# genjax-dev/genjax

Measured on AMD Instinct MI355X. Metric: particles/sec (particle-steps/s), bootstrap SMC sweep, linear-Gaussian SSM T=100, higher is better.
Workload: dtype f32; 1 GPU; BASELINE config 2: linear-Gaussian state-space (T=100), bootstrap SMC, systematic resampling every step; particles_per_gpu=1000000, particles_total=1000000, T=100, resampler=systematic, graph=True, key=314159

## Files before the change

### genjax_amd/csrc/gmx_jit.h

```cpp
#pragma once
#include "gmx_block.h"
#include "gmx_vm.h"
#include "gmx_peer.h"
#if defined(GMX_JIT_RS)
#include "gmx_offspring.h"
#endif
#if defined(GMX_JIT_SH)
#include "gmx_shard_fill.h"
#endif

#if defined(GMX_JIT_BACKGROUND)
#define GMX_JIT_PRIO
#define GMX_JIT_NAME gmx_jit_background_kernel
#else
#define GMX_JIT_PRIO GMX_SETPRIO
#define GMX_JIT_NAME gmx_jit_kernel
#endif

#if defined(GMX_JIT_RS_LOOP)
#define GMX_JIT_BLK gmx_blk
#define GMX_RS_LOOP_MAX 16
#else
#define GMX_JIT_BLK blockIdx.x
#endif

template <int NDYN, int PPV>
struct gmx_jit_ctx {
  const uint32_t* consts;
  const gmx_run_args* A;
  float* lds4;
  uint64_t* lds8;
  float red_x[PPV];
  int cur;
  uint32_t blk;
  uint32_t part;
  uint32_t rows;
  int64_t n_rows;
  float acc_max;
  uint64_t* peer_land;
  uint32_t peer_tag;
  bool first, last;
  __device__ __forceinline__ uint32_t pool(uint32_t i) const {
    return i < (uint32_t)NDYN ? A->uni[i] : consts[i - (uint32_t)NDYN];
  }
  __device__ __forceinline__ const void* in_ptr(uint32_t s) const { return A->in_d[s]; }
  __device__ __forceinline__ void* out_ptr(uint32_t s) const { return A->out_d[s]; }
  __device__ __forceinline__ const void* tab_ptr(uint32_t s) const { return A->tab_d[s]; }
  __device__ __forceinline__ void red_max(float x, bool active) {
    const float m = active ? x : -gmx_inf();
    red_x[cur] = m;
    acc_max = first ? m : gmx_rmax(acc_max, m);
    if (last) {
      const float bm = block_max(acc_max, lds4);
      if (threadIdx.x == 0 && A->red_out_d) A->red_out_d[blk] = bm;
      if (PPV == 4 && A->tile_agg_d) {
        const float ref = gmx_tile_ref(gmx_tile_exp(bm));
        uint64_t s = 0;
#pragma unroll
        for (int p = 0; p < PPV; ++p) s += gmx_exp_fixed(red_x[p] - ref, A->tile_shift);
        s = wave_sum_u64(s);
        if ((threadIdx.x & 63) == 0) lds8[threadIdx.x >> 6] = s;
        __syncthreads();
        const uint64_t a_b = (lds8[0] + lds8[1]) + (lds8[2] + lds8[3]);
        if (threadIdx.x == 0) A->tile_agg_d[blk] = a_b;
        if (peer_land) gmx_peer_put_tile(peer_land, peer_tag, A->peer.world, A->peer.tiles, A->peer.rank, (int)blk, a_b, bm);
      }
    }
  }
  __device__ __forceinline__ void red_lse(float x, bool active) {
    gmx_red_lse(A->red_out_d, lds4, part, rows, x, active);
  }
};

#if defined(GMX_JIT_SH)
#define GMX_JIT_OCC __attribute__((amdgpu_waves_per_eu(1, 4)))
#else
#define GMX_JIT_OCC
#endif
#if defined(GMX_JIT_RS_LOOP)
#define GMX_JIT_LOOP_OPEN                                                                        \
    const int gmx_tiles = (int)((n + (int64_t)(PP * GMX_BLOCK) - 1) / (int64_t)(PP * GMX_BLOCK)); \
    const int gmx_G = (int)gridDim.x;                                                            \
    const int gmx_C = (gmx_tiles + gmx_G - 1) / gmx_G;                                           \
    if (PP == 4 && A.rs.lw_d) {                                                                  \
      __shared__ uint64_t gmx_pf[GMX_RS_LOOP_MAX];                                               \
      uint64_t gmx_tot, gmx_mk;                                                                  \
      gmx_tile_table_pass(A.rs.tile_max_d, A.rs.tile_agg_d, gmx_tiles, (int)blockIdx.x, gmx_G, gmx_C, gmx_pf, gmx_tot, gmx_mk); \
      GMX_JIT_NOUNROLL for (int gmx_c = 0; gmx_c < gmx_C; ++gmx_c) {                             \
        const int gmx_tile = (int)blockIdx.x + gmx_c * gmx_G;                                    \
        if (gmx_tile < gmx_tiles)                                                                \
          gmx_offspring_tile_body<GMX_RESAMPLE_SYSTEMATIC, 0, true>(A.rs.key0, A.rs.key1, A.rs.u0, A.rs.lw_d, A.rs.tile_max_d, \
              (const uint64_t*)nullptr, n, gmx_tiles, gmx_pow2i(A.rs.shift), A.rs.max_out_d, A.rs.total_out_d, \
              const_cast<int32_t*>(A.ancestors_d), nullptr, A.rs.tag, gmx_tile, gmx_pf[gmx_c], gmx_tot, gmx_mk); \
        __syncthreads();                                                                         \
      }                                                                                          \
    }                                                                                            \
    GMX_JIT_NOUNROLL for (int gmx_lc = 0; gmx_lc < gmx_C; ++gmx_lc) {                            \
      const uint32_t gmx_blk = blockIdx.x + (uint32_t)gmx_lc * (uint32_t)gmx_G;                  \
      if ((int)gmx_blk >= gmx_tiles) break;                                   \
      if (gmx_lc) __syncthreads();
#define GMX_JIT_LOOP_CLOSE }
#else
#define GMX_JIT_LOOP_OPEN
#define GMX_JIT_LOOP_CLOSE
#endif
#define GMX_JIT_BEGIN(NREGS, FULLV, NDYN, PPV, NPRE)                                             \
  extern "C" __global__ void __launch_bounds__(GMX_BLOCK) GMX_JIT_OCC GMX_JIT_NAME(int64_t n, const gmx_run_args A) { \
 GMX_JIT_PRIO                                                                                 \
    __shared__ float lds4[4];                                                                    \
    __shared__ uint64_t lds8[4];                                                                 \
    constexpr int PP = PPV;                                                                      \
    typedef gmx_regs_vgpr<NREGS> regs_t;                                                         \
    typedef gmx_jit_ctx<NDYN, PPV> ctx_t;                                                        \
    constexpr bool full_v = FULLV;                                                               \
    ctx_t ctx;                                                                                   \
    ctx.consts = GMX_JIT_CONST; ctx.A = &A; ctx.lds4 = lds4; ctx.lds8 = lds8; ctx.part = 0; ctx.cur = 0; \
    ctx.rows = (uint32_t)((n + GMX_BLOCK - 1) / GMX_BLOCK); ctx.n_rows = n;      \
    ctx.peer_land = nullptr; ctx.peer_tag = 0u;                                                  \
    if (PPV == 4 && A.peer.land_d) {                                         \
      ctx.peer_tag = *A.peer.tag_base_d + (uint32_t)A.peer.step;                                 \
      if (threadIdx.x < (uint32_t)A.peer.world && (int)threadIdx.x != A.peer.rank)               \
        ctx.peer_land = (uint64_t*)A.peer.land_d[threadIdx.x];                                   \
    }                                                                                            \
    GMX_JIT_LOOP_OPEN                                                                            \
    ctx.blk = GMX_JIT_BLK;                                                                       \
    regs_t R[PP];                                                                                \
      \
    const uint32_t n32 = (uint32_t)n;                                                            \
    int64_t idx[PP];                                                                             \
    uint32_t cidx[PP];          \
    uint32_t arow[PP];                                                      \
    uint32_t pre[(NPRE) > 0 ? (NPRE) : 1][PP];                                                   \
    bool act[PP];                                                                                \
    uint32_t gmx_t = 0u;        \
    uint32_t gmx_t0 = 0u, gmx_tf = 0u;    \
               \
    const uint32_t row0 = blockIdx.y * n32;                                                      \
    _Pragma("unroll") for (int p = 0; p < PP; ++p) {                                             \
      R[p].init();                                                                               \
      const uint32_t i32 = (GMX_JIT_BLK * (uint32_t)PP + (uint32_t)p) * (uint32_t)GMX_BLOCK + threadIdx.x; \
      idx[p] = (int64_t)(row0 + i32);                                                            \
      act[p] = i32 < n32;                                                                        \
      cidx[p] = row0 + (act[p] ? i32 : n32 - 1u);                                                \
      arow[p] = 0u;                                                                              \
    }                                                                                            \
    (void)cidx; (void)arow; (void)pre; (void)gmx_t; (void)gmx_t0; (void)gmx_tf;

#define GMX_JIT_POLL_ANC(TAG, STATUS, LIMIT)                                                     \
      const uint32_t* gmx_aw = reinterpret_cast<const uint32_t*>(A.ancestors_d);                 \
      uint32_t gmx_av[PP];                                                                       \
      bool gmx_ok = true;                                                                        \
      _Pragma("unroll") for (int p = 0; p < PP; ++p) {                                           \
        gmx_av[p] = __hip_atomic_load(gmx_aw + cidx[p], __ATOMIC_RELAXED, __HIP_MEMORY_SCOPE_AGENT); \
        gmx_ok &= (gmx_av[p] >> GMX_ANC_TAG_SHIFT) == (TAG);                                     \
      }                                                                                          \
      if (!gmx_ok) {                                                                             \
        const uint64_t gmx_t0 = wall_clock64();                                                  \
        do {                                                                                     \
          __builtin_amdgcn_s_sleep(1);                                                           \
          gmx_ok = true;                                                                         \
          _Pragma("unroll") for (int p = 0; p < PP; ++p) {                                       \
            gmx_av[p] = __hip_atomic_load(gmx_aw + cidx[p], __ATOMIC_RELAXED, __HIP_MEMORY_SCOPE_AGENT); \
            gmx_ok &= (gmx_av[p] >> GMX_ANC_TAG_SHIFT) == (TAG);                                 \
          }                                                                                      \
        } while (!gmx_ok && wall_clock64() - gmx_t0 < 200000000ull);                             \
        if (!gmx_ok) __hip_atomic_store((STATUS), 1ull, __ATOMIC_RELAXED, __HIP_MEMORY_SCOPE_AGENT); \
      }                                                                                          \
      _Pragma("unroll") for (int p = 0; p < PP; ++p) {                                           \
        const uint32_t gmx_i = gmx_av[p] & GMX_ANC_INDEX_MASK;                                   \
        arow[p] = gmx_i < (LIMIT) ? gmx_i : (LIMIT) - 1u;                                        \
      }

#if defined(GMX_JIT_SH)
#define GMX_JIT_PRE_ANC                                                                          \
    if (PP == 4 && A.sh.lw_d) {                                                                  \
      shard_peer gmx_sp;                                                                         \
      gmx_sp.land = (uint64_t* const*)A.sh.peer.land_d; gmx_sp.tag_base = A.sh.peer.tag_base_d;  \
      gmx_sp.status = A.sh.peer.status_d; gmx_sp.step = A.sh.peer.step; gmx_sp.leaves = A.sh.peer.leaves; \
      gmx_sp.state = (const uint32_t* const*)A.sh.state_d; gmx_sp.tail = (uint32_t* const*)A.sh.tail_d;   \
      gmx_shard_fill_body<GMX_RESAMPLE_SYSTEMATIC, true, true, true>(                            \
          A.sh.key0, A.sh.key1, A.sh.u0, A.sh.lw_d, (const uint8_t*)A.sh.stats_own_d, (size_t)0, A.sh.peer.tiles, \
          gmx_pow2i(A.sh.shift), A.sh.peer.rank, A.sh.peer.world, (int32_t)n, (int32_t)A.sh.peer.capacity, A.sh.plan_d, \
          A.sh.total_out_d, A.sh.max_out_d, (const uint32_t*)nullptr, (uint32_t*)nullptr,         \
          const_cast<int32_t*>(A.ancestors_d), gmx_sp, A.sh.tag);                                 \
      const uint32_t gmx_lim = n32 + (uint32_t)A.sh.peer.world * (uint32_t)A.sh.peer.capacity;   \
      GMX_JIT_POLL_ANC(A.sh.tag, A.sh.status_d, gmx_lim)                                         \
       \
    } else {                                                                                     \
      _Pragma("unroll") for (int p = 0; p < PP; ++p) arow[p] = (uint32_t)A.ancestors_d[cidx[p]]; \
    }
#elif defined(GMX_JIT_RS_LOOP)
#define GMX_JIT_PRE_ANC                                                                          \
    if (PP == 4 && A.rs.lw_d) {                                                                  \
      GMX_JIT_POLL_ANC(A.rs.tag, A.rs.status_d, n32)                                             \
    } else {                                                                                     \
      _Pragma("unroll") for (int p = 0; p < PP; ++p) arow[p] = (uint32_t)A.ancestors_d[cidx[p]]; \
    }
#elif defined(GMX_JIT_RS)
#define GMX_JIT_PRE_ANC                                                                          \
    if (PP == 4 && A.rs.lw_d) {                                                                  \
      gmx_offspring_tile_body<GMX_RESAMPLE_SYSTEMATIC, 4, true>(A.rs.key0, A.rs.key1, A.rs.u0, A.rs.lw_d, A.rs.tile_max_d, \
          A.rs.tile_agg_d, n, (int)gridDim.x, gmx_pow2i(A.rs.shift), A.rs.max_out_d, A.rs.total_out_d,          \
          const_cast<int32_t*>(A.ancestors_d), nullptr, A.rs.tag);                                \
      GMX_JIT_POLL_ANC(A.rs.tag, A.rs.status_d, n32)                                             \
    } else {                                                                                     \
      _Pragma("unroll") for (int p = 0; p < PP; ++p) arow[p] = (uint32_t)A.ancestors_d[cidx[p]]; \
    }
#else
#define GMX_JIT_PRE_ANC                                                                          \
    _Pragma("unroll") for (int p = 0; p < PP; ++p) arow[p] = (uint32_t)A.ancestors_d[cidx[p]];
#endif

#define GMX_JIT_PRE_LOAD(K, SLOT, U8, ROW)                                                       \
    _Pragma("unroll") for (int p = 0; p < PP; ++p)                                               \
      pre[K][p] = (U8) ? (uint32_t)((const uint8_t*)A.in_d[SLOT])[ROW[p]] : ((const uint32_t*)A.in_d[SLOT])[ROW[p]];
#define GMX_JIT_PRE(K, SLOT, U8) GMX_JIT_PRE_LOAD(K, SLOT, U8, cidx)
#define GMX_JIT_PRE_G(K, SLOT, U8) GMX_JIT_PRE_LOAD(K, SLOT, U8, arow)
#define GMX_JIT_FENCE __builtin_amdgcn_sched_barrier(0);

#define GMX_JIT_LDPRE(DST, K)                                                                    \
    _Pragma("unroll") for (int p = 0; p < PP; ++p) R[p].set(DST, pre[K][p]);

#define GMX_JIT_OP(W0, W1)                                                                       \
    _Pragma("unroll") for (int p = 0; p < PP; ++p) {                                             \
      ctx.part = GMX_JIT_BLK * PP + p; ctx.first = (p == 0); ctx.last = (p == PP - 1); ctx.cur = p; \
      gmx_vm_step<regs_t, full_v, gmx_cword<W0, W1>, ctx_t>(R[p], gmx_cword<W0, W1>(), idx[p], act[p], A, ctx, gmx_t, gmx_tf); \
    }

#define GMX_JIT_NOUNROLL _Pragma("clang loop unroll(disable)")
#define GMX_JIT_LOOP(COUNT) GMX_JIT_NOUNROLL for (gmx_t0 = 0u; gmx_t0 < (COUNT); ++gmx_t0) { gmx_t = gmx_t0; gmx_tf = gmx_t0;
#define GMX_JIT_ENDLOOP } gmx_t = 0u; gmx_t0 = 0u; gmx_tf = 0u;
#define GMX_JIT_LOOP2(COUNT) GMX_JIT_NOUNROLL for (uint32_t gmx_t1 = 0u; gmx_t1 < (COUNT); ++gmx_t1) { gmx_t = gmx_t1; gmx_tf = gmx_t0 * (COUNT) + gmx_t1;
#define GMX_JIT_ENDLOOP2 } gmx_t = gmx_t0; gmx_tf = gmx_t0;
#define GMX_JIT_LOOP3(COUNT) { const uint32_t gmx_tp = gmx_t, gmx_tfp = gmx_tf;                  \
    GMX_JIT_NOUNROLL for (uint32_t gmx_t2 = 0u; gmx_t2 < (COUNT); ++gmx_t2) { gmx_t = gmx_t2; gmx_tf = gmx_tfp * (COUNT) + gmx_t2;
#define GMX_JIT_ENDLOOP3 } gmx_t = gmx_tp; gmx_tf = gmx_tfp; }

#define GMX_JIT_END GMX_JIT_LOOP_CLOSE }
```

### genjax_amd/csrc/gmx_kernels.hip

```cpp
#include <hip/hip_runtime.h>
#include <hip/hiprtc.h>
#include <stdio.h>
#include <stdlib.h>
#include <string.h>
#include <sys/stat.h>
#include <unistd.h>

#include <new>
#include <atomic>
#include <string>
#include <vector>

#include "gmx_block.h"
#include "gmx_vm.h"
#include "gmx_resample.h"
#include "gmx_peer.h"
#include "gmx_sorted.h"
#include "gmx_offspring.h"
#include "gmx_shard_fill.h"

static thread_local char g_err[512] = "";

static int gmx_fail(const char* fmt, const char* a = "", long long b = 0) {
  snprintf(g_err, sizeof(g_err), fmt, a, b);
// ... 144 lines not shown
      case OP_LOOP: ok = loop_depth < 3 && w1 >= 1u; ++loop_depth; in_loop = true; P.uses_loop = true; break;
      case OP_ENDLOOP: ok = loop_depth > 0; --loop_depth; in_loop = loop_depth > 0; break;
      case OP_UNI: ok = D(dst) && w1 < P.n_uni; break;
      case OP_LDIN:
        ok = D(dst) && a < P.n_in && (!(b & GMX_F_IDX) || (R(c) && !(b & (GMX_F_STEP | GMX_F_FLAT | GMX_F_BCAST))));
        if (b & GMX_F_GATHER) P.uses_gather = true;
        break;
      case OP_LDTAB: ok = D(dst) && R(b) && a < P.n_tab; break;
      case OP_STOUT: ok = R(b) && a < P.n_out; break;
      case OP_LDKEY: ok = R2(dst); P.uses_key = true; break;
      case OP_KDERIVE: ok = R2(dst) && R2(a); break;
      case OP_KDERIVER: ok = R2(dst) && R2(a) && R(b); break;
      case OP_KSPLITU: ok = R2(dst) && R(a) && R(b); break;
      case OP_MOV: case OP_NEG: case OP_ABS: case OP_EXP: case OP_LOG: case OP_LOG1P:
      case OP_SQRT: case OP_SIN: case OP_COS: case OP_TANH: case OP_SIGMOID:
      case OP_SOFTPLUS: case OP_FLOOR: case OP_CEIL: case OP_ROUND: case OP_LGAMMA:
      case OP_SQUARE: case OP_RECIP: case OP_NOT: case OP_I2F: case OP_F2I: case OP_INEG:
        ok = D(dst) && R(a); break;
      case OP_ADD: case OP_SUB: case OP_MUL: case OP_DIV: case OP_MIN: case OP_MAX: case OP_POW:
      case OP_FLT: case OP_FLE: case OP_FGT: case OP_FGE: case OP_FEQ: case OP_FNE:
      case OP_IEQ: case OP_INE: case OP_ILT: case OP_ILE: case OP_IGT: case OP_IGE:
      case OP_AND: case OP_OR: case OP_XOR: case OP_IADD: case OP_ISUB: case OP_IMUL:
        ok = D(dst) && R(a) && R(b); break;
      case OP_SEL: ok = D(dst) && R(a) && R(b) && R(c); break;
      case OP_S_NORMAL: case OP_S_UNIFORM: case OP_S_BETA:
        ok = D(dst) && R(a) && R(b) && R2(c); break;
      case OP_S_FLIP: case OP_S_BERNL: case OP_S_LOGGAMMA: ok = D(dst) && R(a) && R2(c); break;
      case OP_S_CATSTEP: ok = R2(dst) && R(a) && R(b) && R2(c); break;
      case OP_L_NORMAL: case OP_L_UNIFORM: case OP_L_BETA:
        ok = D(dst) && R(a) && R(b) && R(c); break;
      case OP_L_FLIP: case OP_L_BERNL: ok = D(dst) && R(a) && R(c); break;
      case OP_REDMAX: case OP_REDLSE:
        ok = R(a); P.uses_red = true;
        if (op == OP_REDLSE) P.uses_lse = true; else ++P.n_redmax;
        break;
      default: ok = false;
    }
    if ((op == OP_LDIN && (b & (GMX_F_STEP | GMX_F_IDX))) || (op == OP_STOUT && (dst & GMX_F_STEP))) {
      P.uses_step = true;
    }
    if (!ok) return gmx_fail("gmx_program_create: invalid instruction%s at pc %lld", "", pc);
  }
  if (in_loop) return gmx_fail("gmx_program_create: OP_LOOP without OP_ENDLOOP%s");
  P.code_h.assign(ins, ins + 2 * (size_t)n_instr);
  P.consts.assign(ins + 2 * (size_t)n_instr, ins + 2 * (size_t)n_instr + n_const);
  return 0;
}

extern "C" int gmx_program_create(const uint32_t* blob, size_t n_words, gmx_program** out) {
  if (!out) return gmx_fail("gmx_program_create: null argument%s");
  gmx_program P;
  if (parse_program(blob, n_words, P)) return 1;
  const uint32_t n_instr = P.n_instr;
  GMX_HIP(hipMalloc((void**)&P.code_d, sizeof(uint32_t) * 2 * (n_instr ? n_instr : 1)));
  if (n_instr)
    GMX_HIP(hipMemcpy(P.code_d, P.code_h.data(), sizeof(uint32_t) * 2 * n_instr, hipMemcpyHostToDevice));
  gmx_program* h = new (std::nothrow) gmx_program(P);
  if (!h) return gmx_fail("gmx_program_create: out of host memory%s");
  *out = h;
  return 0;
}

extern "C" int gmx_program_destroy(gmx_program* p) {
  if (!p) return 0;
  if (p->code_d) (void)hipFree(p->code_d);
  if (p->jit_module) (void)hipModuleUnload(p->jit_module);
  delete p;
  return 0;
}


#include "gmx_embed.inc"

static bool jit_enabled() {
  const char* e = getenv("GENMI_JIT");
  return !(e && e[0] == '0');
}

static int jit_pp_for(const gmx_program* p) {
  return (p->n_regs <= 16 && p->n_instr <= 96 && !p->uses_lse) ? 4 : 1;
}

#define JIT_MAX_PRE 8
static std::string jit_source(const gmx_program* p, bool* gathers_prefetched = nullptr) {
  std::string s = p->background ? "#define GMX_JIT_BACKGROUND 1\n" : "";
  if (const char* f_ = getenv("GENMI_JIT_FAULT")) { if (f_[0] == '1') s += "#define GMX_JIT_FAULT 1\n"; }
  if (p->fuse_rs) s += "#define GMX_JIT_RS 1\n";
  if (p->fuse_rs_loop) s += "#define GMX_JIT_RS_LOOP 1\n";
  if (p->fuse_sh) s += "#define GMX_JIT_SH 1\n";
  s += "#include \"gmx_jit.h\"\n";
  char buf[128];
  s += "__device__ static constexpr uint32_t GMX_JIT_CONST[] = {";
  for (size_t k = 0; k < p->consts.size(); ++k) { snprintf(buf, sizeof(buf), "0x%08xu,", p->consts[k]); s += buf; }
  s += "0u};\n";
  struct pre_t { uint32_t slot, flags; };
  std::vector<pre_t> pres;
  std::vector<int> pre_of(p->n_instr, -1);
  bool any_gather = false;
  uint32_t first_gather_pc = p->n_instr, first_key_pc = p->n_instr;
  bool fits = true, seen_loop = false;
  for (uint32_t pc = 0; pc < p->n_instr && fits; ++pc) {
    const uint32_t w0 = p->code_h[2 * pc], op = w0 & 0xffu, a = (w0 >> 16) & 0xffu, b = w0 >> 24;
    if ((op == OP_LDKEY || op == OP_KDERIVE) && first_key_pc == p->n_instr && !seen_loop) first_key_pc = pc;
    if (op == OP_LOOP) seen_loop = true;
    if (op != OP_LDIN || (b & (GMX_F_BCAST | GMX_F_STEP | GMX_F_IDX))) continue;
    int k = -1;
    for (size_t j = 0; j < pres.size(); ++j)
      if (pres[j].slot == a && pres[j].flags == b) k = (int)j;
    if (k < 0) {
      if (pres.size() == JIT_MAX_PRE) { fits = false; break; }
      k = (int)pres.size();
      pres.push_back({a, b});
    }
    pre_of[pc] = k;
    if (b & GMX_F_GATHER) { any_gather = true; if (pc < first_gather_pc) first_gather_pc = pc; }
  }
  if (const char* e_ = getenv("GENMI_JIT_NOPRE")) { if (e_[0] == '1' && !p->fuse_rs && !p->fuse_sh) fits = false; }
  if (!fits) { pres.clear(); pre_of.assign(p->n_instr, -1); any_gather = false; }
  if (gathers_prefetched) {
    *gathers_prefetched = any_gather;
    for (uint32_t pc = 0; pc < p->n_instr; ++pc) {
      const uint32_t w0 = p->code_h[2 * pc];
      if ((w0 & 0xffu) == OP_LDIN && ((w0 >> 24) & GMX_F_GATHER) && pre_of[pc] < 0) *gathers_prefetched = false;
    }
  }
  const uint32_t gpos = (any_gather && first_key_pc < first_gather_pc) ? first_key_pc + 1 : 0;
  snprintf(buf, sizeof(buf), "GMX_JIT_BEGIN(%u, %s, %u, %d, %d)\n", p->n_regs < 16 ? 16u : (p->n_regs < 32 ? 32u : 64u),
           p->needs_full ? "true" : "false", p->n_dyn, jit_pp_for(p), (int)pres.size());
  s += buf;
  if (any_gather) s += "  GMX_JIT_PRE_ANC\n";
  for (size_t k = 0; k < pres.size(); ++k)
    if (!(pres[k].flags & GMX_F_GATHER)) {
      snprintf(buf, sizeof(buf), "  GMX_JIT_PRE(%d, %u, %d)\n", (int)k, pres[k].slot, (pres[k].flags & GMX_F_U8) ? 1 : 0);
      s += buf;
    }
  auto gathers = [&]() {
    for (size_t k = 0; k < pres.size(); ++k)
      if (pres[k].flags & GMX_F_GATHER) {
        snprintf(buf, sizeof(buf), "  GMX_JIT_PRE_G(%d, %u, %d)\n", (int)k, pres[k].slot, (pres[k].flags & GMX_F_U8) ? 1 : 0);
        s += buf;
      }
    s += "  GMX_JIT_FENCE\n";
  };
  if (!pres.empty()) s += "  GMX_JIT_FENCE\n";
  if (any_gather && gpos == 0) gathers();
  int jit_depth = 0;
  for (uint32_t pc = 0; pc < p->n_instr; ++pc) {
    const uint32_t op_ = p->code_h[2 * pc] & 0xffu;
    if (op_ == OP_LOOP) {
      static const char* const open_[3] = {"  GMX_JIT_LOOP(%uu)\n", "  GMX_JIT_LOOP2(%uu)\n", "  GMX_JIT_LOOP3(%uu)\n"};
      snprintf(buf, sizeof(buf), open_[jit_depth < 2 ? jit_depth : 2], p->code_h[2 * pc + 1]);
      ++jit_depth;
    } else if (op_ == OP_ENDLOOP) {
      static const char* const close_[3] = {"  GMX_JIT_ENDLOOP\n", "  GMX_JIT_ENDLOOP2\n", "  GMX_JIT_ENDLOOP3\n"};
      --jit_depth;
      snprintf(buf, sizeof(buf), "%s", close_[jit_depth < 2 ? (jit_depth < 0 ? 0 : jit_depth) : 2]);
    }
    else if (pre_of[pc] >= 0)
      snprintf(buf, sizeof(buf), "  GMX_JIT_LDPRE(%u, %d)\n", (p->code_h[2 * pc] >> 8) & 0xffu, pre_of[pc]);
    else
      snprintf(buf, sizeof(buf), "  GMX_JIT_OP(0x%08xu, 0x%08xu)\n", p->code_h[2 * pc], p->code_h[2 * pc + 1]);
    s += buf;
    if (any_gather && gpos == pc + 1) gathers();
  }
  s += "GMX_JIT_END\n";
  return s;
}

extern "C" int gmx_program_is_specialized(const gmx_program* p) { return p && p->jit_fn ? 1 : 0; }
static std::atomic<int64_t> g_jit_rejected{0};
extern "C" int64_t gmx_jit_rejected_count(void) { return g_jit_rejected.load(); }
extern "C" int gmx_program_despecialize(gmx_program* p, const char* why) {
  if (!p) return gmx_fail("gmx_program_despecialize: null program%s");
  if (!p->jit_fn) return 0;
  (void)hipDeviceSynchronize();
  (void)hipModuleUnload(p->jit_module);
  p->jit_fn = nullptr; p->jit_module = nullptr; p->jit_code_hash = 0;
  ++g_jit_rejected;
  (void)gmx_fail("specialised kernel rejected, the interpreter takes over: %s", why ? why : "");
  return 0;
}
extern "C" uint64_t gmx_program_code_hash(const gmx_program* p) { return p && p->jit_fn ? p->jit_code_hash : 0ull; }
extern "C" int gmx_program_writes_tile_stats(const gmx_program* p) {
  return p && p->jit_fn && p->jit_pp == 4 && p->n_redmax == 1 && !p->uses_lse ? 1 : 0;
}

extern "C" int gmx_program_set_fuse_resample(gmx_program* p) {
  if (!p) return gmx_fail("gmx_program_set_fuse_resample: null program%s");
  if (p->jit_fn) return gmx_fail("gmx_program_set_fuse_resample: the program is already specialised%s");
  p->fuse_rs = true;
  return 0;
}
extern "C" int gmx_program_set_fuse_resample_loop(gmx_program* p) {
  if (!p) return gmx_fail("gmx_program_set_fuse_resample_loop: null program%s");
  if (p->jit_fn) return gmx_fail("gmx_program_set_fuse_resample_loop: the program is already specialised%s");
  p->fuse_rs = true;
  p->fuse_rs_loop = true;
  return 0;
}
static int64_t rs_loop_grid(const gmx_program* p, int64_t tiles) {
  int64_t g = p->jit_resident_blocks > 0 ? p->jit_resident_blocks : 256;
  if (g > 1024) g = 1024;

  return tiles < g ? tiles : g;
}
extern "C" int gmx_program_fuses_resample(const gmx_program* p) {
  return p && p->jit_fn && p->fuse_rs && p->jit_pp == 4 && p->uses_gather && p->jit_gathers_pre ? 1 : 0;
}
extern "C" int gmx_program_set_fuse_shard_step(gmx_program* p) {
  if (!p) return gmx_fail("gmx_program_set_fuse_shard_step: null program%s");
  if (p->jit_fn) return gmx_fail("gmx_program_set_fuse_shard_step: the program is already specialised%s");
  p->fuse_sh = true;
  return 0;
}
extern "C" int gmx_program_fuses_shard_step(const gmx_program* p) {
  return p && p->jit_fn && p->fuse_sh && p->jit_pp == 4 && p->uses_gather && p->jit_gathers_pre ? 1 : 0;
}
extern "C" int64_t gmx_program_resident_particles(const gmx_program* p) {
// ... 190 lines not shown
  }
  size_t cs = 0;
  if (rc == HIPRTC_SUCCESS) {
    hiprtcGetCodeSize(prog, &cs);
    if (code_out && code_cap >= cs) hiprtcGetCode(prog, code_out);
  }
  hiprtcDestroyProgram(&prog);
  return cs;
}

extern "C" int64_t gmx_program_grid(const gmx_program* p, int64_t n) {
  int64_t per = GMX_BLOCK;
  if (p && p->jit_fn && !p->uses_lse) per = (int64_t)GMX_BLOCK * p->jit_pp;
  return (n + per - 1) / per;
}

static int peer_check(const char* who, const gmx_peer& P, int64_t n_per_rank);
extern "C" int gmx_program_run(const gmx_program* p, int64_t n, const gmx_run_args* args,
                               gmx_stream stream) {
  if (!p || !args) return gmx_fail("gmx_program_run: null argument%s");
  if (n < 0) return gmx_fail("gmx_program_run: negative n%s");
  if (n == 0) return 0;
  if (n > (int64_t)0x7fffffff * GMX_BLOCK) return gmx_fail("gmx_program_run: n too large%s");
  for (uint32_t s = 0; s < p->n_in; ++s)
    if (!args->in_d[s]) return gmx_fail("gmx_program_run: input slot %s%lld is null", "", s);
  for (uint32_t s = 0; s < p->n_out; ++s)
    if (!args->out_d[s]) return gmx_fail("gmx_program_run: output slot %s%lld is null", "", s);
  for (uint32_t s = 0; s < p->n_tab; ++s)
    if (!args->tab_d[s]) return gmx_fail("gmx_program_run: table slot %s%lld is null", "", s);
  if (p->uses_gather && !args->ancestors_d)
    return gmx_fail("gmx_program_run: program gathers but ancestors_d is null%s");
  const bool fused_rs = args->rs.lw_d != nullptr;
  if (fused_rs) {
    const gmx_resample_in& q = args->rs;
    if (!gmx_program_fuses_resample(p))
      return gmx_fail("gmx_program_run: rs is set but this program cannot resample in its own launch "
                      "(gmx_program_set_fuse_resample before specialising; 4 particles per thread; gathering)%s");
    if (!q.tile_max_d || !q.tile_agg_d || !q.max_out_d || !q.total_out_d || !q.status_d)
      return gmx_fail("gmx_program_run: rs has a null pointer%s");
    if ((uintptr_t)q.lw_d & 15) return gmx_fail("gmx_program_run: rs.lw_d must be 16-byte aligned%s");
    if ((!p->fuse_rs_loop && (n + RS_TILE - 1) / RS_TILE > 1024) || n > gmx_program_resident_particles(p) ||
        n > (int64_t)GMX_ANC_INDEX_MASK + 1)
      return gmx_fail("gmx_program_run: rs: every workgroup of the launch must be resident at once (n <= 2^20 and "
                      "n <= gmx_program_resident_particles(); a looped program — gmx_program_set_fuse_resample_loop — "
                      "walks up to 16 tiles per workgroup: n <= 2^24)%s");
    if (q.shift < 1 || q.shift > 62) return gmx_fail("gmx_program_run: rs.shift out of range%s");
    int need = 0;
    while (((int64_t)1 << need) < n) ++need;
    if (q.shift + need > 62) return gmx_fail("gmx_program_run: rs.shift too large for n (overflow)%s");
    if (q.tag < 1u || q.tag > GMX_ANC_TAG_MAX) return gmx_fail("gmx_program_run: rs.tag must be in [1, 255]%s");
    if (args->tile_agg_d == q.tile_agg_d || (const float*)args->red_out_d == q.tile_max_d)
      return gmx_fail("gmx_program_run: rs reads the tile statistics this launch writes (use two sets)%s");
    for (uint32_t s = 0; s < p->n_out; ++s)
      if ((const void*)args->out_d[s] == (const void*)q.lw_d)
        return gmx_fail("gmx_program_run: rs.lw_d is also an output of this launch (use two buffers)%s");
  }
  const bool fused_sh = args->sh.lw_d != nullptr;
  if (fused_sh) {
    const gmx_shard_in& q = args->sh;
    if (fused_rs) return gmx_fail("gmx_program_run: rs and sh are both set%s");
    if (!gmx_program_fuses_shard_step(p))
      return gmx_fail("gmx_program_run: sh is set but this program cannot route a sharded step in its own launch "
                      "(gmx_program_set_fuse_shard_step before specialising; 4 particles per thread; gathering)%s");
    if (!q.stats_own_d || !q.plan_d || !q.total_out_d || !q.max_out_d || !q.status_d)
      return gmx_fail("gmx_program_run: sh has a null pointer%s");
    if (((uintptr_t)q.lw_d & 15) || ((uintptr_t)q.stats_own_d & 7))
      return gmx_fail("gmx_program_run: sh.lw_d must be 16-byte and sh.stats_own_d 8-byte aligned%s");
    if (peer_check("gmx_program_run (sh)", q.peer, n)) return 1;
    if (q.peer.world > 8 || (int64_t)q.peer.world * q.peer.tiles > 4 * GMX_BLOCK)
      return gmx_fail("gmx_program_run: sh: world <= 8 and world * tiles <= 1024%s");
    if (n + (int64_t)q.peer.world * q.peer.capacity > (int64_t)GMX_ANC_INDEX_MASK + 1)
      return gmx_fail("gmx_program_run: sh: n + world * capacity must fit the 21-bit index of an ancestor word%s");
    if (n > gmx_program_resident_particles(p))
      return gmx_fail("gmx_program_run: sh: every workgroup of the launch must be resident at once "
                      "(n <= gmx_program_resident_particles())%s");
    if (q.shift < 1 || q.shift > 62) return gmx_fail("gmx_program_run: sh.shift out of range%s");
    if (q.tag < 1u || q.tag > GMX_ANC_TAG_MAX) return gmx_fail("gmx_program_run: sh.tag must be in [1, 255]%s");
    for (int l = 0; l < q.peer.leaves; ++l)
      if (!q.state_d[l] || !q.tail_d[l]) return gmx_fail("gmx_program_run: sh: a leaf pointer is null%s");
    for (uint32_t s_ = 0; s_ < p->n_out; ++s_)
      if ((const void*)args->out_d[s_] == (const void*)q.lw_d)
        return gmx_fail("gmx_program_run: sh.lw_d is also an output of this launch (use two buffers)%s");
  }
  if (p->uses_red && !args->red_out_d)
    return gmx_fail("gmx_program_run: program reduces but red_out_d is null%s");
  if (args->tile_agg_d) {
    if (!gmx_program_writes_tile_stats(p))
      return gmx_fail("gmx_program_run: tile_agg_d is set but this program cannot write tile statistics "
                      "(gmx_program_writes_tile_stats)%s");
    if (args->tile_shift < 1 || args->tile_shift > 62) return gmx_fail("gmx_program_run: tile_shift out of range%s");
  }
  if (p->uses_step && args->step_stride < n)
    return gmx_fail("gmx_program_run: step_stride must be at least n for a program with step-indexed leaves%s");
  if (p->uses_key) {
    int km = args->key_mode;
    if (km != GMX_KEY_ARRAY && km != GMX_KEY_SPLIT && km != GMX_KEY_ROWSPLIT && km != GMX_KEY_BCAST)
      return gmx_fail("gmx_program_run: program draws but key_mode is unset%s");
    if ((km == GMX_KEY_ARRAY || km == GMX_KEY_ROWSPLIT) && !args->keys_d)
      return gmx_fail("gmx_program_run: keys_d is null%s");
    if (km == GMX_KEY_ROWSPLIT && args->key_inner <= 0)
      return gmx_fail("gmx_program_run: key_inner must be positive%s");
  }
  dim3 grid((unsigned)((n + GMX_BLOCK - 1) / GMX_BLOCK)), block(GMX_BLOCK);
  hipStream_t st = (hipStream_t)stream;
  gmx_run_args patched;
  if (p->n_const || fused_rs || fused_sh) {
    patched = *args;
    for (uint32_t k = 0; k < p->n_const; ++k) patched.uni[p->n_dyn + k] = p->consts[k];
    if (fused_rs) {
      uint32_t b0, b1;
      gmx_threefry2x32(patched.rs.key0, patched.rs.key1, 0u, 0u, &b0, &b1);
      patched.rs.u0 = (b0 ^ b1) >> 9;
    }
    if (fused_sh) {
      uint32_t b0, b1;
      gmx_threefry2x32(patched.sh.key0, patched.sh.key1, 0u, 0u, &b0, &b1);
      patched.sh.u0 = (b0 ^ b1) >> 9;
    }
    args = &patched;
  }
  if (p->jit_fn) {
    if (n >= 0x7fffffffLL - 4 * GMX_BLOCK)
      return gmx_fail("gmx_program_run: a specialised kernel indexes particles with 32 bits (n < 2^31 - 1024)%s");
    struct { int64_t n; gmx_run_args A; } ka;
    ka.n = n; ka.A = *args;
    size_t ka_size = sizeof(ka);
    void* config[] = {HIP_LAUNCH_PARAM_BUFFER_POINTER, &ka, HIP_LAUNCH_PARAM_BUFFER_SIZE, &ka_size,
                      HIP_LAUNCH_PARAM_END};
    int64_t rows = 1, per_row = n;
    if (p->background && args->key_mode == GMX_KEY_ROWSPLIT && args->key_inner > 0 && n % args->key_inner == 0 &&
        n / args->key_inner > 1 && n / args->key_inner <= 65535 && p->n_in == 0 && !p->uses_red && !p->uses_step) {
      rows = n / args->key_inner;
      per_row = args->key_inner;
      ka.n = per_row;
    }
    unsigned jgrid = (unsigned)((per_row + (int64_t)GMX_BLOCK * p->jit_pp - 1) / ((int64_t)GMX_BLOCK * p->jit_pp));
    if (p->fuse_rs_loop && p->jit_pp == 4) jgrid = (unsigned)rs_loop_grid(p, (int64_t)jgrid);
    const unsigned dyn_lds = p->lds_pad;
    GMX_HIP(hipModuleLaunchKernel(p->jit_fn, jgrid, (unsigned)rows, 1, GMX_BLOCK, 1, 1, dyn_lds, st, nullptr, config));
    return 0;
  }
  if (p->n_regs > 31)
    return gmx_fail("gmx_program_run: a program with more than 31 live values runs only as a specialised kernel "
                    "(gmx_program_specialize; hiprtc unavailable or GENMI_JIT=0?)%s");
  if (p->n_regs <= 15) {
    if (p->needs_full)
      hipLaunchKernelGGL((k_vm<gmx_regs_vgpr<16>, true>), grid, block, 0, st, p->code_d, p->n_instr, n, *args);
    else
      hipLaunchKernelGGL(k_vm_lean, grid, block, 0, st, p->code_d, p->n_instr, n, *args);
  } else {
    if (p->needs_full)
      hipLaunchKernelGGL((k_vm<gmx_regs_vgpr<32>, true>), grid, block, 0, st, p->code_d, p->n_instr, n, *args);
    else
      hipLaunchKernelGGL((k_vm<gmx_regs_vgpr<32>, false>), grid, block, 0, st, p->code_d, p->n_instr, n, *args);
  }
  GMX_HIP(hipGetLastError());
  return 0;
}

__global__ void __launch_bounds__(GMX_BLOCK)
k_split(uint32_t k0, uint32_t k1, int64_t n, int64_t off, uint32_t* __restrict__ out) {
  int64_t i = (int64_t)blockIdx.x * GMX_BLOCK + threadIdx.x;
  if (i >= n) return;
  gmx_key k; k.k0 = k0; k.k1 = k1;
  gmx_key o = gmx_split_child(k, (uint64_t)(off + i));
  reinterpret_cast<uint2*>(out)[i] = make_uint2(o.k0, o.k1);
// ... 2539 lines not shown
```

### genjax_amd/csrc/gmx_offspring.h

```cpp
#pragma once
#include "gmx_block.h"
#include "gmx_resample.h"
#include "gmx_sorted.h"

#define CDF_VEC_OT 4
#ifndef RS_THREADS
#define RS_THREADS 256
#endif
#define RS_TILE (RS_THREADS * CDF_VEC_OT)
#ifndef RS_MAX_TILES
#define RS_MAX_TILES 2048
#endif
static_assert(RS_TILE == 1024 && RS_THREADS == GMX_BLOCK, "resampling tiles are the CDF's definition tiles");
static_assert(RS_MAX_TILES % GMX_BLOCK == 0, "tile table shape");

#define GMX_ANC_TAG_SHIFT 24
#define GMX_ANC_INDEX_MASK 0xffffffu
#define GMX_ANC_TAG_MAX 255u
__device__ __forceinline__ void gmx_store_u32x4_sc1(uint32_t* p, uint32_t a, uint32_t b, uint32_t c, uint32_t d) {
  typedef uint32_t v4 __attribute__((ext_vector_type(4)));
  v4 v; v.x = a; v.y = b; v.z = c; v.w = d;
  asm volatile("s_nop 1\n\tglobal_store_dwordx4 %0, %1, off sc1\n\ts_nop 1" :: "v"(p), "v"(v) : "memory");
}
__device__ __forceinline__ void gmx_store_u32_sc1(uint32_t* p, uint32_t a) {
  __hip_atomic_store(p, a, __ATOMIC_RELAXED, __HIP_MEMORY_SCOPE_AGENT);
}

typedef uint32_t rs_u32x4_a4 __attribute__((ext_vector_type(4), aligned(4)));
typedef uint32_t sorted_u32x2_a4 __attribute__((ext_vector_type(2), aligned(4)));
struct sorted_ctx {
  const uint32_t* slow; const uint32_t* guide; const uint64_t* toff;
  uint64_t stot, gmax; uint32_t sh, mask; double ratio;
};
__device__ __forceinline__ sorted_ctx sorted_ctx_of(const uint32_t* table, int64_t n, uint64_t total, uint64_t stot, uint32_t sh) {
  const gmx_sorted_layout L = gmx_sorted_layout_of(n);
  sorted_ctx X;
  X.slow = table; X.guide = table + L.off_guide;
  X.toff = reinterpret_cast<const uint64_t*>(table + L.off_toff);
  X.stot = stot;
  X.sh = sh;
  X.mask = (1u << X.sh) - 1u;
  X.gmax = X.stot >> X.sh;
  X.ratio = (double)X.stot / (double)(total ? total : 1ull);
  return X;
}
__device__ __forceinline__ int64_t sorted_below_exact(const sorted_ctx& X, uint64_t c, uint64_t total, int64_t j, int64_t n) {
  const u128 R = mul64(c, X.stot);
  j = j < 0 ? 0 : (j > n ? n : j);
  auto below = [&](int64_t k) {
    const uint64_t off = X.toff[k >> 10];
    const uint64_t S = off + (uint64_t)(uint32_t)(X.slow[k] - (uint32_t)off);
    return gt128(R, mul64(S, total));
  };
  while (j > 0 && !below(j - 1)) --j;
  while (j < n && below(j)) ++j;
  return j;
}

#define RS_TPB 1
#define RS_BLOCK (GMX_BLOCK * RS_TPB)
#define RS_WAVES (RS_BLOCK / GMX_WAVE)
static_assert(RS_MAX_TILES % RS_BLOCK == 0, "tile table shape");
#define RS_FILL_SLOTS 2048
template <int kind, int PER, bool TAGGED>
__device__ __forceinline__ void
gmx_offspring_tile_body(uint32_t k0, uint32_t k1, uint32_t u0_host, const float* __restrict__ lw,
                        const float* __restrict__ tmax, const uint64_t* __restrict__ agg, int64_t n, int n_tiles, float scale,
                        float* __restrict__ max_out, uint64_t* __restrict__ total_out, int32_t* __restrict__ anc,
                        const uint32_t* __restrict__ uslot, uint32_t tag,
                        int tile0 = -1, uint64_t a_prefix = 0ull, uint64_t a_total = 0ull, uint64_t a_mk = 0ull) {
  const int blk = tile0 >= 0 ? tile0 : (int)blockIdx.x;
  const uint32_t tagw = TAGGED ? (tag << GMX_ANC_TAG_SHIFT) : 0u;
  __shared__ uint64_t s_below[RS_WAVES], s_all[RS_WAVES], s_scan[RS_WAVES], s_g[RS_TPB];
  __shared__ float s_max[RS_WAVES];
  const int lane = threadIdx.x & 63, wave = threadIdx.x >> 6;
  const int grp = threadIdx.x >> 8, ltid = threadIdx.x & (GMX_BLOCK - 1);
  const int first_tile = blk * RS_TPB;
  const int my_tile = first_tile + grp;
  const bool tile_ok = my_tile < n_tiles;
  const int tile_c = tile_ok ? my_tile : n_tiles - 1;
  const int64_t i0 = (int64_t)tile_c * RS_TILE + (int64_t)ltid * CDF_VEC_OT;
  float x[CDF_VEC_OT];
  const bool full_tile = (int64_t)(tile_c + 1) * RS_TILE <= n;
  if (full_tile) {
    float4 v = *reinterpret_cast<const float4*>(lw + i0);
    x[0] = v.x; x[1] = v.y; x[2] = v.z; x[3] = v.w;
  } else {
#pragma unroll
    for (int c = 0; c < CDF_VEC_OT; ++c) {
      const int64_t ic = i0 + c < n ? i0 + c : n - 1;
      const float xv = lw[ic];
      x[c] = (i0 + c < n) ? xv : -gmx_inf();
    }
  }
  constexpr bool PREF = (PER == 0);
  constexpr int PERN = PREF ? 1 : PER;
  static_assert(PER >= 0 && PER * RS_BLOCK <= RS_MAX_TILES, "rows of the tile table per thread");
  static_assert(!PREF || RS_TPB == 1, "the prefix form works on one tile per block");
  uint64_t ta[PERN];
  float tm[PERN];
  uint64_t pf_prefix = 0, pf_total = 0, pf_mk = 0;
  if (PREF) {
    if (agg) { pf_prefix = agg[tile_c]; pf_total = agg[n_tiles]; pf_mk = agg[n_tiles + 1]; }
    else { pf_prefix = a_prefix; pf_total = a_total; pf_mk = a_mk; }
  } else {
#pragma unroll
    for (int r = 0; r < PERN; ++r) {
      ta[r] = 0ull; tm[r] = -gmx_inf();
      if (r * RS_BLOCK < n_tiles) {
        const int t = r * RS_BLOCK + (int)threadIdx.x;
        const int tc = t < n_tiles ? t : n_tiles - 1;
        ta[r] = agg[tc];
        tm[r] = tmax[tc];
      }
    }
  }
  const float tmax_mine = tmax[tile_c];
  uint64_t sx_stot = 0; uint32_t sx_sh = 0;
  if constexpr (kind == GMX_RESAMPLE_MULTINOMIAL_SORTED) {
    const gmx_sorted_layout L = gmx_sorted_layout_of(n);
    sx_stot = reinterpret_cast<const uint64_t*>(uslot + L.off_toff)[L.tiles];
    sx_sh = uslot[L.off_sh];
  }
  __builtin_amdgcn_sched_barrier(0);
  if (!PREF) {
#pragma unroll
    for (int r = 0; r < PERN; ++r) {
      const int t = r * RS_BLOCK + (int)threadIdx.x;
      ta[r] = (t < n_tiles) ? ta[r] : 0ull;
      tm[r] = (t < n_tiles) ? tm[r] : -gmx_inf();
    }
  }
  const int32_t k_b = gmx_tile_exp(tmax_mine);
  const float ref_b = gmx_tile_ref(k_b);
  float M = -gmx_inf();
  if (PREF) {
    M = gmx_u2f((uint32_t)pf_mk);
  } else {
#pragma unroll
    for (int r = 0; r < PERN; ++r)
      if (r * RS_BLOCK < n_tiles) M = gmx_rmax(M, tm[r]);
    M = wave_max(M);
  }
  uint64_t q[CDF_VEC_OT];
  uint64_t run = 0;
#pragma unroll
  for (int c = 0; c < CDF_VEC_OT; ++c) {
    const uint64_t w = weight_fixed(x[c], ref_b, scale);
    run += (tile_ok && i0 + c < n) ? w : 0ull;
    q[c] = run;
  }
  const uint64_t inc = wave_scan_u64(run);
  if (!PREF && lane == 0) s_max[wave] = M;
  if (lane == 63) s_scan[wave] = inc;
  __syncthreads();
  if (!PREF) {
    M = s_max[0];
#pragma unroll
    for (int w = 1; w < RS_WAVES; ++w) M = gmx_rmax(M, s_max[w]);
  }
  uint64_t wave_off = 0;
#pragma unroll
  for (int w = 0; w < 4; ++w) wave_off += (w < (wave & 3)) ? s_scan[4 * grp + w] : 0ull;
  const uint64_t loc = wave_off + (inc - run);
  const int32_t K = PREF ? (int32_t)(uint32_t)(pf_mk >> 32) : gmx_tile_exp(M);
  uint64_t prefix = 0, total = 0;
  if (PREF) {
    prefix = pf_prefix; total = pf_total;
  } else {
    uint64_t below = 0, all = 0;
#pragma unroll
    for (int r = 0; r < PERN; ++r) {
      if (r * RS_BLOCK < n_tiles) {
        const int t = r * RS_BLOCK + (int)threadIdx.x;
        const uint64_t G = gmx_tile_scale(ta[r], gmx_tile_exp(tm[r]), K);
        all += G;
        below += (t < first_tile) ? G : 0ull;
        if (t >= first_tile && t < first_tile + RS_TPB) s_g[t - first_tile] = G;
      }
    }
    below = wave_sum_u64(below);
    all = wave_sum_u64(all);
    if (lane == 0) { s_below[wave] = below; s_all[wave] = all; }
    __syncthreads();
#pragma unroll
    for (int w = 0; w < RS_WAVES; ++w) { prefix += s_below[w]; total += s_all[w]; }
#pragma unroll
    for (int j = 0; j < RS_TPB; ++j) prefix += (j < grp) ? s_g[j] : 0ull;
  }
  if (blk == 0 && threadIdx.x == 0) { *total_out = total; *max_out = M; }
  if (!tile_ok) return;
  gmx_key key; key.k0 = k0; key.k1 = k1;
  if (total == 0) {
#pragma unroll
    for (int c = 0; c < CDF_VEC_OT; ++c)
      if (i0 + c < n) {
        if (TAGGED) gmx_store_u32_sc1(reinterpret_cast<uint32_t*>(anc) + (i0 + c), (uint32_t)(n - 1) | tagw);
        else anc[i0 + c] = (int32_t)(n - 1);
      }
    return;
  }
  const double n_over_total = (double)n / (double)total;
  const double eps = (double)n * 0x1p-44 + 0x1p-40;
  const int32_t n32 = (int32_t)n;
  uint64_t cv[CDF_VEC_OT + 1];
  cv[0] = prefix + gmx_tile_scale(loc, k_b, K);
#pragma unroll
// ... 214 lines not shown
```

Baseline: 71.10 billion particle-steps/s.

## Preload hot kernel arguments into SGPRs and specialise JIT kernel without peer exchange

Adds an X-macro list that loads frequently used kernel arguments (buffer pointers, keys, sizes) into scalar registers at kernel entry behind a scheduling barrier, so later scalar loads from the argument segment are avoided. It compiles out the peer-exchange setup and per-tile peer put when the program is single-GPU resample-fused, and adds a host check that rejects peer use in that case. It also reorders the resample prologue after the non-gather prefetches, computes the tile count from n instead of gridDim, and rewrites the log-weight load in the offspring tile body as a speculative float4 plus scalar tail. The cost is more SGPR pressure and extra specialisation paths.

```diff
diff --git a/genjax_amd/csrc/gmx_jit.h b/genjax_amd/csrc/gmx_jit.h
--- a/genjax_amd/csrc/gmx_jit.h
+++ b/genjax_amd/csrc/gmx_jit.h
@@ -22,6 +22,43 @@
 #define GMX_RS_LOOP_MAX 16
 #else
 #define GMX_JIT_BLK blockIdx.x
+#endif
+
+#ifndef GMX_JIT_HOT_PROGRAM
+#define GMX_JIT_HOT_PROGRAM(X)
+#endif
+#if defined(GMX_JIT_RS_LOOP)
+#define GMX_JIT_HOT_GRID(X) X(grid, (uint32_t)gridDim.x)
+#else
+#define GMX_JIT_HOT_GRID(X)
+#endif
+#if defined(GMX_JIT_RS)
+#define GMX_JIT_HOT_RS(X)                                                                        \
+    X(rs_lw, A.rs.lw_d) X(rs_tmax, A.rs.tile_max_d) X(rs_agg, A.rs.tile_agg_d) X(rs_max, A.rs.max_out_d) \
+    X(rs_tot, A.rs.total_out_d) X(rs_status, A.rs.status_d) X(rs_shift, A.rs.shift) X(rs_tag, A.rs.tag) \
+    X(rs_k0, A.rs.key0) X(rs_k1, A.rs.key1) X(rs_u0, A.rs.u0) GMX_JIT_HOT_GRID(X)
+#else
+#define GMX_JIT_HOT_RS(X)
+#endif
+#if defined(GMX_JIT_RS) && !defined(GMX_JIT_SH)
+#define GMX_JIT_HOT_LIST(X)                                                                      \
+    X(n, n) X(anc, A.ancestors_d) X(red, A.red_out_d) X(agg, A.tile_agg_d) X(tshift, A.tile_shift) \
+    GMX_JIT_HOT_RS(X) GMX_JIT_HOT_PROGRAM(X)
+#else
+#define GMX_JIT_HOT_LIST(X)
+#endif
+#define GMX_JIT_HOT_LOAD(TAG, EXPR) const auto gmx_hot_##TAG = (EXPR);
+#define GMX_JIT_HOT_PIN(TAG, EXPR) asm volatile("" :: "s"(gmx_hot_##TAG));
+
+#if defined(GMX_JIT_PEER)
+#define GMX_JIT_PEER_SETUP(PPV)                                                                  \
+    if (PPV == 4 && A.peer.land_d) {                                         \
+      ctx.peer_tag = *A.peer.tag_base_d + (uint32_t)A.peer.step;                                 \
+      if (threadIdx.x < (uint32_t)A.peer.world && (int)threadIdx.x != A.peer.rank)               \
+        ctx.peer_land = (uint64_t*)A.peer.land_d[threadIdx.x];                                   \
+    }
+#else
+#define GMX_JIT_PEER_SETUP(PPV)
 #endif
 
 template <int NDYN, int PPV>
@@ -63,7 +100,9 @@
         __syncthreads();
         const uint64_t a_b = (lds8[0] + lds8[1]) + (lds8[2] + lds8[3]);
         if (threadIdx.x == 0) A->tile_agg_d[blk] = a_b;
+#if defined(GMX_JIT_PEER)
         if (peer_land) gmx_peer_put_tile(peer_land, peer_tag, A->peer.world, A->peer.tiles, A->peer.rank, (int)blk, a_b, bm);
+#endif
       }
     }
   }
@@ -107,6 +146,9 @@
 #define GMX_JIT_BEGIN(NREGS, FULLV, NDYN, PPV, NPRE)                                             \
   extern "C" __global__ void __launch_bounds__(GMX_BLOCK) GMX_JIT_OCC GMX_JIT_NAME(int64_t n, const gmx_run_args A) { \
  GMX_JIT_PRIO                                                                                 \
+    GMX_JIT_HOT_LIST(GMX_JIT_HOT_LOAD)                                                           \
+    __builtin_amdgcn_sched_barrier(0);                                                           \
+    GMX_JIT_HOT_LIST(GMX_JIT_HOT_PIN)                                                            \
     __shared__ float lds4[4];                                                                    \
     __shared__ uint64_t lds8[4];                                                                 \
     constexpr int PP = PPV;                                                                      \
@@ -117,11 +159,7 @@
     ctx.consts = GMX_JIT_CONST; ctx.A = &A; ctx.lds4 = lds4; ctx.lds8 = lds8; ctx.part = 0; ctx.cur = 0; \
     ctx.rows = (uint32_t)((n + GMX_BLOCK - 1) / GMX_BLOCK); ctx.n_rows = n;      \
     ctx.peer_land = nullptr; ctx.peer_tag = 0u;                                                  \
-    if (PPV == 4 && A.peer.land_d) {                                         \
-      ctx.peer_tag = *A.peer.tag_base_d + (uint32_t)A.peer.step;                                 \
-      if (threadIdx.x < (uint32_t)A.peer.world && (int)threadIdx.x != A.peer.rank)               \
-        ctx.peer_land = (uint64_t*)A.peer.land_d[threadIdx.x];                                   \
-    }                                                                                            \
+    GMX_JIT_PEER_SETUP(PPV)                                                                      \
     GMX_JIT_LOOP_OPEN                                                                            \
     ctx.blk = GMX_JIT_BLK;                                                                       \
     regs_t R[PP];                                                                                \
@@ -200,7 +238,8 @@
 #define GMX_JIT_PRE_ANC                                                                          \
     if (PP == 4 && A.rs.lw_d) {                                                                  \
       gmx_offspring_tile_body<GMX_RESAMPLE_SYSTEMATIC, 4, true>(A.rs.key0, A.rs.key1, A.rs.u0, A.rs.lw_d, A.rs.tile_max_d, \
-          A.rs.tile_agg_d, n, (int)gridDim.x, gmx_pow2i(A.rs.shift), A.rs.max_out_d, A.rs.total_out_d,          \
+          A.rs.tile_agg_d, n, (int)((n + (int64_t)(RS_TILE - 1)) / (int64_t)RS_TILE) , \
+          gmx_pow2i(A.rs.shift), A.rs.max_out_d, A.rs.total_out_d,                                \
           const_cast<int32_t*>(A.ancestors_d), nullptr, A.rs.tag);                                \
       GMX_JIT_POLL_ANC(A.rs.tag, A.rs.status_d, n32)                                             \
     } else {                                                                                     \
diff --git a/genjax_amd/csrc/gmx_kernels.hip b/genjax_amd/csrc/gmx_kernels.hip
--- a/genjax_amd/csrc/gmx_kernels.hip
+++ b/genjax_amd/csrc/gmx_kernels.hip
@@ -250,14 +250,38 @@
 }
 
 #define JIT_MAX_PRE 8
+static bool jit_has_peer(const gmx_program* p) { return p->fuse_sh || !p->fuse_rs; }
 static std::string jit_source(const gmx_program* p, bool* gathers_prefetched = nullptr) {
   std::string s = p->background ? "#define GMX_JIT_BACKGROUND 1\n" : "";
   if (const char* f_ = getenv("GENMI_JIT_FAULT")) { if (f_[0] == '1') s += "#define GMX_JIT_FAULT 1\n"; }
   if (p->fuse_rs) s += "#define GMX_JIT_RS 1\n";
   if (p->fuse_rs_loop) s += "#define GMX_JIT_RS_LOOP 1\n";
   if (p->fuse_sh) s += "#define GMX_JIT_SH 1\n";
+  if (jit_has_peer(p)) s += "#define GMX_JIT_PEER 1\n";
+  char buf[128];
+  if (p->fuse_rs && !p->fuse_sh) {
+    int left = 40;
+    s += "#define GMX_JIT_HOT_PROGRAM(X)";
+    auto hot = [&](const char* tag, unsigned k, const char* expr) {
+      if (left <= 0) return;
+      --left;
+      snprintf(buf, sizeof(buf), expr, k);
+      char item[192];
+      snprintf(item, sizeof(item), " X(%s%u, %s)", tag, k, buf);
+      s += item;
+    };
+    for (uint32_t k = 0; k < p->n_in; ++k) hot("in", k, "A.in_d[%u]");
+    for (uint32_t k = 0; k < p->n_out; ++k) hot("out", k, "A.out_d[%u]");
+    for (uint32_t k = 0; k < p->n_tab; ++k) hot("tab", k, "A.tab_d[%u]");
+    for (uint32_t k = 0; k < p->n_dyn; ++k) hot("uni", k, "A.uni[%u]");
+    if (p->uses_key) {
+      hot("key", 0, "A.key_mode"); hot("key", 1, "A.key0"); hot("key", 2, "A.key1"); hot("key", 3, "A.keys_d");
+      hot("key", 4, "A.key_inner"); hot("key", 5, "A.index_offset");
+    }
+    if (p->uses_step) hot("step", 0, "A.step_stride");
+    s += "\n";
+  }
   s += "#include \"gmx_jit.h\"\n";
-  char buf[128];
   s += "__device__ static constexpr uint32_t GMX_JIT_CONST[] = {";
   for (size_t k = 0; k < p->consts.size(); ++k) { snprintf(buf, sizeof(buf), "0x%08xu,", p->consts[k]); s += buf; }
   s += "0u};\n";
@@ -296,12 +320,12 @@
   snprintf(buf, sizeof(buf), "GMX_JIT_BEGIN(%u, %s, %u, %d, %d)\n", p->n_regs < 16 ? 16u : (p->n_regs < 32 ? 32u : 64u),
            p->needs_full ? "true" : "false", p->n_dyn, jit_pp_for(p), (int)pres.size());
   s += buf;
-  if (any_gather) s += "  GMX_JIT_PRE_ANC\n";
   for (size_t k = 0; k < pres.size(); ++k)
     if (!(pres[k].flags & GMX_F_GATHER)) {
       snprintf(buf, sizeof(buf), "  GMX_JIT_PRE(%d, %u, %d)\n", (int)k, pres[k].slot, (pres[k].flags & GMX_F_U8) ? 1 : 0);
       s += buf;
     }
+  if (any_gather) s += "  GMX_JIT_PRE_ANC\n";
   auto gathers = [&]() {
     for (size_t k = 0; k < pres.size(); ++k)
       if (pres[k].flags & GMX_F_GATHER) {
@@ -658,6 +682,9 @@
       if ((const void*)args->out_d[s_] == (const void*)q.lw_d)
         return gmx_fail("gmx_program_run: sh.lw_d is also an output of this launch (use two buffers)%s");
   }
+  if (args->peer.land_d && p->jit_fn && !jit_has_peer(p))
+    return gmx_fail("gmx_program_run: peer is set but this program asked for the single-GPU resample-first prologue "
+                    "(gmx_program_set_fuse_resample): its kernel is specialised without the peer exchange%s");
   if (p->uses_red && !args->red_out_d)
     return gmx_fail("gmx_program_run: program reduces but red_out_d is null%s");
   if (args->tile_agg_d) {
diff --git a/genjax_amd/csrc/gmx_offspring.h b/genjax_amd/csrc/gmx_offspring.h
--- a/genjax_amd/csrc/gmx_offspring.h
+++ b/genjax_amd/csrc/gmx_offspring.h
@@ -74,25 +74,20 @@
   __shared__ uint64_t s_below[RS_WAVES], s_all[RS_WAVES], s_scan[RS_WAVES], s_g[RS_TPB];
   __shared__ float s_max[RS_WAVES];
   const int lane = threadIdx.x & 63, wave = threadIdx.x >> 6;
-  const int grp = threadIdx.x >> 8, ltid = threadIdx.x & (GMX_BLOCK - 1);
+  const int grp = RS_TPB == 1 ? 0 : (int)(threadIdx.x >> 8), ltid = threadIdx.x & (GMX_BLOCK - 1);
   const int first_tile = blk * RS_TPB;
   const int my_tile = first_tile + grp;
   const bool tile_ok = my_tile < n_tiles;
   const int tile_c = tile_ok ? my_tile : n_tiles - 1;
   const int64_t i0 = (int64_t)tile_c * RS_TILE + (int64_t)ltid * CDF_VEC_OT;
-  float x[CDF_VEC_OT];
-  const bool full_tile = (int64_t)(tile_c + 1) * RS_TILE <= n;
-  if (full_tile) {
-    float4 v = *reinterpret_cast<const float4*>(lw + i0);
-    x[0] = v.x; x[1] = v.y; x[2] = v.z; x[3] = v.w;
-  } else {
-#pragma unroll
-    for (int c = 0; c < CDF_VEC_OT; ++c) {
-      const int64_t ic = i0 + c < n ? i0 + c : n - 1;
-      const float xv = lw[ic];
-      x[c] = (i0 + c < n) ? xv : -gmx_inf();
-    }
-  }
+  static_assert(CDF_VEC_OT == 4, "one float4 of log-weights per thread");
+  const bool whole = i0 + 3 < n;
+  float4 xl = make_float4(0.0f, 0.0f, 0.0f, 0.0f);
+  float xs[3] = {-gmx_inf(), -gmx_inf(), -gmx_inf()};
+  if (whole) xl = *reinterpret_cast<const float4*>(lw + i0);
+#pragma unroll
+  for (int c = 0; c < 3; ++c)
+    if (!whole && i0 + c < n) xs[c] = lw[i0 + c];
   constexpr bool PREF = (PER == 0);
   constexpr int PERN = PREF ? 1 : PER;
   static_assert(PER >= 0 && PER * RS_BLOCK <= RS_MAX_TILES, "rows of the tile table per thread");
@@ -123,6 +118,10 @@
     sx_sh = uslot[L.off_sh];
   }
   __builtin_amdgcn_sched_barrier(0);
+  uint32_t whole_v = whole ? 1u : 0u;
+  asm volatile("" : "+v"(whole_v));
+  const bool wh = whole_v != 0u;
+  const float x[CDF_VEC_OT] = {wh ? xl.x : xs[0], wh ? xl.y : xs[1], wh ? xl.z : xs[2], wh ? xl.w : -gmx_inf()};
   if (!PREF) {
 #pragma unroll
     for (int r = 0; r < PERN; ++r) {
```

Result: no change. 71.26 billion particle-steps/s, median of 3 (+0.2%).
